# A2R-Lab/GBD-PCG

Measured on AMD Instinct MI355X. Metric: PCG iterations/sec and GB/s on block-tridiag SpMV, stateSize×knotPoints, higher is better.
Workload: dtype f32

## Files before the change

### gbd-pcg_amd/csrc/api.hip

```cpp
#include <hip/hip_runtime.h>

#include <cstdio>
#include <cstring>
#include <new>
#include <vector>

#include "../../include/gbdpcg.h"
#include "internal.hpp"

#ifndef GBDPCG_KKT_SKIP_L
#define GBDPCG_KKT_SKIP_L 1
#endif

using namespace gbdpcg;

struct gbdpcg_context {
    DeviceInfo dev;
    gbdpcg_path forced = GBDPCG_PATH_AUTO;
    int symmetric = 2;
    uint8_t *sym_flags = nullptr;
    size_t sym_cap = 0;
    hipError_t last_err = hipSuccess;
    uint32_t *d_iters = nullptr;
    uint8_t *d_exit = nullptr;
    uint32_t *h_iters = nullptr;
    uint8_t *h_exit = nullptr;
    uint32_t *h_done = nullptr;
    uint32_t *h_done_dev = nullptr;
    uint32_t *h_iters_dev = nullptr;
    uint8_t *h_exit_dev = nullptr;
    void *ws = nullptr;
    size_t ws_bytes = 0;
    struct PersistWs {
        uint64_t key;
        void *buf;
    };
    std::vector<PersistWs> pws;
    void *cluster_ws = nullptr;
    void *cluster_rescue = nullptr;
    void *pws_last = nullptr;
    std::vector<void *> retired;
};

struct gbdpcg_graph {
    gbdpcg_handle_t h = nullptr;
    hipGraph_t graph = nullptr;
    hipGraphExec_t exec = nullptr;
};

namespace gbdpcg {

template <typename T> int choose_vec(uint32_t n, const void *const *ptrs, int nptrs)
{
    const int cand[3] = {4, 2, 1};
// ... 174 lines not shown
    return grow_buffer(h, reinterpret_cast<void **>(&h->sym_flags), &h->sym_cap, batch);
}

template <typename T>
gbdpcg_status solve_impl(gbdpcg_handle_t h, uint32_t n, uint32_t N, uint32_t batch, const T *d_S, const T *d_Pinv,
                         const T *d_gamma, T *d_lambda, T *d_r, T *d_p, T tol, uint32_t max_iter,
                         uint32_t *d_iters, uint8_t *d_exit, hipStream_t stream, bool blocking = false,
                         uint32_t given_verdict_stride = 0, bool known_symmetric = false)
{
    if (!h || !d_S || !d_gamma || !d_lambda || !d_iters || !shape_ok(n, N, batch)) return GBDPCG_ERR_INVALID;
    if (!mappable<T>(n)) return GBDPCG_ERR_UNSUPPORTED;
    PcgArgs<T> a{d_S, d_Pinv, d_gamma, d_lambda, d_r, d_p, tol, max_iter, n, N, batch, d_iters, d_exit};
    a.cluster_ws = h->cluster_ws;
    a.rescue_vec = h->cluster_rescue;
    DEVICE_SCOPE(h);
    if (const uint32_t per = persist_slices<T>(h, n, N, batch, max_iter)) {
        const size_t ms = (size_t)3 * n * n * N, vs = (size_t)n * N;
        for (uint32_t b0 = 0; b0 < batch; b0 += per) {
            const uint32_t nb = batch - b0 < per ? batch - b0 : per;
            const gbdpcg_status st = solve_impl<T>(h, n, N, nb, d_S + b0 * ms, d_Pinv ? d_Pinv + b0 * ms : nullptr, d_gamma + b0 * vs,
                                                   d_lambda + b0 * vs, d_r ? d_r + b0 * vs : nullptr, d_p ? d_p + b0 * vs : nullptr, tol,
                                                   max_iter, d_iters + b0, d_exit ? d_exit + b0 : nullptr, stream);
            if (st != GBDPCG_OK) return st;
        }
        return GBDPCG_OK;
    }
    const gbdpcg_path path = pick_path<T>(h, n, N, batch);
    if (path == GBDPCG_PATH_PERSISTENT || path == GBDPCG_PATH_PERSISTENT_1R) {
        hipStreamCaptureStatus cs = hipStreamCaptureStatusNone;
        const bool capturing = hipStreamIsCapturing(stream, &cs) == hipSuccess && cs != hipStreamCaptureStatusNone;
        void *pws = nullptr;
        gbdpcg_status st = get_pws(h, sizeof(T), n, N, batch, persist_total_bytes<T>(h, n, N, batch), !capturing, &pws);
        if (st != GBDPCG_OK) return st;
        a.rescue_vec = static_cast<unsigned char *>(pws) + persist_rescue_offset<T>(n, N, batch);
        HIP_TRY(h, launch_pcg_persist<T>(h->dev, a, pws, stream, path == GBDPCG_PATH_PERSISTENT_1R));
    } else if (path == GBDPCG_PATH_FUSED) {
        const bool cluster_only = cluster_members<T>(n, N) != 0 && !resident_sym_shape<T>(n, N);
        bool has_sym = h->symmetric != 0 && d_Pinv != nullptr && !cluster_only && fused_has_symmetric<T>(h->dev, n, N, batch);
        const uint32_t members = cluster_members<T>(n, N);
        const bool one_cluster_round = members != 0 && (uint64_t)batch * members <= (uint64_t)h->dev.num_cus &&
                                       max_iter < (1u << 18) &&
                                       !(reinterpret_cast<uintptr_t>(d_S) % 8) && !(d_Pinv && reinterpret_cast<uintptr_t>(d_Pinv) % 8);
        if (h->symmetric == 2 && one_cluster_round) has_sym = false;
        if (has_sym && h->symmetric == 2 && known_symmetric) {
            a.symmetric = true;
            HIP_TRY(h, launch_pcg_fused<T>(h->dev, a, stream));
        } else if (has_sym && h->symmetric == 2 && given_verdict_stride) {
            a.sel_stride = given_verdict_stride;
            a.sel = h->sym_flags;
            a.symmetric = true;
            a.want = 1;
            HIP_TRY(h, launch_pcg_fused<T>(h->dev, a, stream));
            a.symmetric = false;
            a.want = 0;
            HIP_TRY(h, launch_pcg_fused<T>(h->dev, a, stream));
        } else if (has_sym && h->symmetric == 2) {
            const uint32_t vpp = check_pair_chunks<T>(n, N);
            const bool aligned16 = !((reinterpret_cast<uintptr_t>(d_S) | reinterpret_cast<uintptr_t>(d_Pinv)) % 16);
            const size_t need_flags = (size_t)batch * (vpp && aligned16 ? vpp : 1);
            if (need_flags > h->sym_cap) {
                hipStreamCaptureStatus cs = hipStreamCaptureStatusNone;
                if (hipStreamIsCapturing(stream, &cs) == hipSuccess && cs != hipStreamCaptureStatusNone)
                    return GBDPCG_ERR_ALLOC;
                gbdpcg_status st = ensure_sym_flags(h, need_flags);
                if (st != GBDPCG_OK) return st;
            }
            hipError_t cerr = hipSuccess;
            uint32_t stride = 1;
            if (vpp && launch_check_symmetric_pair<T>(n, N, batch, d_S, d_Pinv, h->sym_flags, stream, &cerr, &stride)) {
                HIP_TRY(h, cerr);
            } else {
                stride = 1;
                HIP_TRY(h, launch_check_symmetric<T>(h->dev, n, N, batch, d_S, h->sym_flags, false, stream));
                HIP_TRY(h, launch_check_symmetric<T>(h->dev, n, N, batch, d_Pinv, h->sym_flags, true, stream));
            }
            a.sel_stride = stride;
            a.sel = h->sym_flags;
            a.symmetric = true;
            a.want = 1;
            HIP_TRY(h, launch_pcg_fused<T>(h->dev, a, stream));
            a.symmetric = false;
            a.want = 0;
            HIP_TRY(h, launch_pcg_fused<T>(h->dev, a, stream));
        } else {
            a.symmetric = has_sym && h->symmetric == 1;
            HIP_TRY(h, launch_pcg_fused<T>(h->dev, a, stream));
        }
    } else {
        const size_t need = split_workspace_bytes<T>(n, N, batch);
        if (need > h->ws_bytes) {
            hipStreamCaptureStatus cs = hipStreamCaptureStatusNone;
            if (hipStreamIsCapturing(stream, &cs) == hipSuccess && cs != hipStreamCaptureStatusNone)
                return GBDPCG_ERR_ALLOC;
            gbdpcg_status st = ensure_ws(h, need);
            if (st != GBDPCG_OK) return st;
        }
        const volatile uint32_t *poll = nullptr;
        if (blocking && h->h_done_dev) {
            h->h_done[0] = 0;
            h->h_done[1] = 0;
            a.host_done = h->h_done_dev;
            poll = h->h_done;
        }
        HIP_TRY(h, launch_pcg_split<T>(h->dev, a, h->ws, stream, poll));
    }
    return GBDPCG_OK;
}

template <typename T>
gbdpcg_status spmv_impl(gbdpcg_handle_t h, uint32_t n, uint32_t N, uint32_t batch, const T *d_M, const T *d_x,
                        T *d_y, hipStream_t stream)
{
    if (!h || !d_M || !d_x || !d_y || !shape_ok(n, N, batch)) return GBDPCG_ERR_INVALID;
    if (!mappable<T>(n)) return GBDPCG_ERR_UNSUPPORTED;
    DEVICE_SCOPE(h);
    SpmvArgs<T> a{d_M, d_x, d_y, n, N, batch};
    a.symmetric = h->symmetric == 1;
    HIP_TRY(h, launch_spmv<T>(h->dev, a, stream));
    return GBDPCG_OK;
}

template <typename T> size_t verdict_bytes(uint32_t n, uint32_t N, uint32_t batch)
{
    const uint32_t a = check_pair_chunks<T>(n, N), b = pinv_verdict_chunks<T>(n, N, GBDPCG_PINV_STAIR);
    const uint32_t m = a > b ? a : b;
    return (size_t)batch * (m ? m : 1);
}

template <typename T>
gbdpcg_status form_pinv_solve_impl(gbdpcg_handle_t h, uint32_t n, uint32_t N, uint32_t batch, const T *d_S, T *d_Pinv,
                                   gbdpcg_pinv_kind kind, const T *d_gamma, T *d_lambda, T *d_r, T *d_p, T tol,
                                   uint32_t max_iter, uint32_t *d_iters, uint8_t *d_exit, hipStream_t stream)
{
    if (!h || !d_S || !d_Pinv || !d_gamma || !d_lambda || !d_iters || !shape_ok(n, N, batch) || (int)kind < 0 ||
        (int)kind > 2)
        return GBDPCG_ERR_INVALID;
    if (!mappable<T>(n)) return GBDPCG_ERR_UNSUPPORTED;
    DEVICE_SCOPE(h);
    uint32_t stride = 0;
    if (h->symmetric == 2 && pick_path<T>(h, n, N, batch) == GBDPCG_PATH_FUSED &&
        fused_has_symmetric<T>(h->dev, n, N, batch))
        stride = pinv_verdict_chunks<T>(n, N, (int)kind);
    if (stride) {
        const size_t need = verdict_bytes<T>(n, N, batch);
        if (need > h->sym_cap) {
            hipStreamCaptureStatus cs = hipStreamCaptureStatusNone;
            if (hipStreamIsCapturing(stream, &cs) == hipSuccess && cs != hipStreamCaptureStatusNone) return GBDPCG_ERR_ALLOC;
            gbdpcg_status st = ensure_sym_flags(h, need);
            if (st != GBDPCG_OK) return st;
        }
    }
    HIP_TRY(h, launch_form_pinv<T>(h->dev, n, N, batch, d_S, d_Pinv, (int)kind, stream, stride ? h->sym_flags : nullptr));
    return solve_impl<T>(h, n, N, batch, d_S, d_Pinv, d_gamma, d_lambda, d_r, d_p, tol, max_iter, d_iters, d_exit, stream,
                         false, stride);
}

template <typename T>
gbdpcg_status solve_blocking_impl(gbdpcg_handle_t h, uint32_t n, uint32_t N, const T *d_S, const T *d_Pinv,
                                  const T *d_gamma, T *d_lambda, T *d_r, T *d_p, T tol, uint32_t max_iter,
                                  uint32_t *h_iters, uint8_t *h_exit)
{
    if (!h) return GBDPCG_ERR_INVALID;
    hipStream_t s = nullptr;
    const bool direct = h->h_iters_dev != nullptr;
    gbdpcg_status st = solve_impl<T>(h, n, N, 1, d_S, d_Pinv, d_gamma, d_lambda, d_r, d_p, tol, max_iter,
                                     direct ? h->h_iters_dev : h->d_iters, direct ? h->h_exit_dev : h->d_exit, s, true);
    if (st != GBDPCG_OK) return st;
    if (!direct) {
        HIP_TRY(h, hipMemcpyAsync(h->h_iters, h->d_iters, sizeof(uint32_t), hipMemcpyDeviceToHost, s));
        HIP_TRY(h, hipMemcpyAsync(h->h_exit, h->d_exit, sizeof(uint8_t), hipMemcpyDeviceToHost, s));
    }
    HIP_TRY(h, hipStreamSynchronize(s));
    if (h_iters) *h_iters = *h->h_iters;
    if (h_exit) *h_exit = *h->h_exit;
    return GBDPCG_OK;
}

template <typename T>
gbdpcg_status solve_host_impl(gbdpcg_handle_t h, uint32_t n, uint32_t N, const T *h_S, const T *h_Pinv,
// ... 612 lines not shown
```

### gbd-pcg_amd/csrc/internal.hpp

```cpp
#pragma once

#include <hip/hip_runtime.h>
#include <stdint.h>
#include <stddef.h>

namespace gbdpcg {

struct DeviceInfo {
    int device = 0;
    int num_cus = 256;
    size_t lds_per_cu = 160 * 1024;
    size_t lds_per_wg_max = 160 * 1024;
};

constexpr uint32_t kItersGaveUp = 0xffffffffu;

template <typename A> __device__ __forceinline__ bool pcg_takes(const A &a, uint32_t prob)
{
    if (!a.sel) return true;
    bool sym = true;
    for (uint32_t c = 0; c < a.sel_stride; ++c) sym &= a.sel[(size_t)prob * a.sel_stride + c] == 1;
    return sym == (a.want == 1);
}

template <typename A>
__device__ __forceinline__ unsigned long long pcg_takes_mask(const A &a, uint32_t first, uint32_t step, uint32_t count, uint32_t lane)
{
    if (!a.sel) return count >= 64 ? ~0ull : ((1ull << count) - 1ull);
    bool mine = false;
    if (lane < count) {
        const size_t prob = (size_t)first + (size_t)lane * step;
        bool sym = true;
        for (uint32_t c = 0; c < a.sel_stride; ++c) sym &= a.sel[prob * a.sel_stride + c] == 1;
        mine = sym == (a.want == 1);
    }
    return __ballot(mine);
}

template <typename T> struct SpmvArgs {
    const T *M;
    const T *x;
    T *y;
    uint32_t n, N, batch;
    bool symmetric = false;
};

template <typename T> struct PcgArgs {
    const T *S;
    const T *Pinv;
    const T *gamma;
    T *lambda;
    T *r;
    T *p;
    T tol;
    uint32_t max_iter;
    uint32_t n, N, batch;
    uint32_t *iters;
    uint8_t *max_iter_exit;
    bool symmetric = false;
    const uint8_t *sel = nullptr;
    uint8_t want = 0;
    uint32_t sel_stride = 1;
    uint32_t *host_done = nullptr;
    void *cluster_ws = nullptr;
    void *rescue_vec = nullptr;
    bool rescue_off = false;
};

template <typename T> int choose_vec(uint32_t n, const void *const *ptrs, int nptrs);

#define GBDPCG_SPECIALIZED_N(X) X(2) X(4) X(6) X(8) X(10) X(12) X(13) X(14) X(16) X(18) X(20) X(24) X(36)

template <typename T, int NCT> constexpr int best_v()
{
    for (int V : {4, 2, 1})
        if ((size_t)V * sizeof(T) <= 16 && NCT % V == 0 && NCT / V <= 64) return V;
    return 1;
}

template <typename T> hipError_t launch_spmv(const DeviceInfo &dev, const SpmvArgs<T> &a, hipStream_t s);

template <typename T> size_t fused_lds_bytes(uint32_t n, uint32_t N, uint32_t waves);
template <typename T> bool fused_fits(const DeviceInfo &dev, uint32_t n, uint32_t N);
template <typename T> hipError_t launch_pcg_fused(const DeviceInfo &dev, const PcgArgs<T> &a, hipStream_t s);

template <typename T> bool resident_shape(uint32_t n, uint32_t N);
template <typename T> void resident_prepare(uint32_t n, uint32_t N);
template <typename T>
bool launch_pcg_resident(const DeviceInfo &dev, const PcgArgs<T> &a, hipStream_t s, hipError_t *err);
template <typename T> bool resident_sym_shape(uint32_t n, uint32_t N);
template <typename T>
bool launch_pcg_resident_sym(const DeviceInfo &dev, const PcgArgs<T> &a, hipStream_t s, hipError_t *err);

template <typename T> uint32_t cluster_members(uint32_t n, uint32_t N);
size_t cluster_workspace_bytes(const DeviceInfo &dev);
size_t cluster_rescue_bytes(const DeviceInfo &dev);
template <typename T>
bool launch_pcg_cluster(const DeviceInfo &dev, const PcgArgs<T> &a, hipStream_t s, hipError_t *err);

template <typename T> size_t split_workspace_bytes(uint32_t n, uint32_t N, uint32_t batch);
template <typename T>
hipError_t launch_pcg_split(const DeviceInfo &dev, const PcgArgs<T> &a, void *workspace, hipStream_t s,
                            const volatile uint32_t *host_done_poll = nullptr);

template <typename T>
uint32_t persist_knots_per_wg(const DeviceInfo &dev, uint32_t n, uint32_t N, uint32_t batch, bool one_reduction = false);
template <typename T> size_t persist_workspace_bytes(uint32_t n, uint32_t N, uint32_t batch);
template <typename T> size_t persist_rescue_bytes(uint32_t n, uint32_t N, uint32_t batch);
template <typename T>
hipError_t launch_pcg_persist(const DeviceInfo &dev, const PcgArgs<T> &a, void *workspace, hipStream_t s,
                              bool one_reduction = false);
template <typename T>
hipError_t launch_pcg_persist_b(const PcgArgs<T> &a, void *workspace, hipStream_t s, bool one_reduction, uint32_t K);
template <typename T>
hipError_t launch_pcg_persist_c(const PcgArgs<T> &a, void *workspace, hipStream_t s, bool one_reduction, uint32_t K);

template <typename T>
hipError_t launch_check_symmetric(const DeviceInfo &dev, uint32_t n, uint32_t N, uint32_t batch, const T *M,
                                  uint8_t *flags, bool and_into, hipStream_t s);
hipError_t launch_fill_bytes(uint8_t *p, uint8_t v, size_t count, hipStream_t s);
hipError_t launch_fill_words(uint32_t *p, uint32_t v, size_t count, hipStream_t s);
template <typename T>
bool launch_check_symmetric_pair(uint32_t n, uint32_t N, uint32_t batch, const T *A, const T *B, uint8_t *flags,
                                 hipStream_t s, hipError_t *err, uint32_t *verdicts_per_problem = nullptr);
template <typename T> uint32_t check_pair_chunks(uint32_t n, uint32_t N);
template <typename T> bool fused_has_symmetric(const DeviceInfo &dev, uint32_t n, uint32_t N, uint32_t batch);

template <typename T>
hipError_t launch_form_pinv(const DeviceInfo &dev, uint32_t n, uint32_t N, uint32_t batch, const T *S,
                            T *Pinv, int kind, hipStream_t s, uint8_t *verdicts = nullptr, bool s_symmetric = false);
template <typename T> uint32_t pinv_verdict_chunks(uint32_t n, uint32_t N, int kind);

template <typename T>
hipError_t launch_form_schur(const DeviceInfo &dev, uint32_t nx, uint32_t nu, uint32_t N, uint32_t batch, const T *G, const T *C,
                             const T *g, const T *c, T *S, T *gamma, T *Ginv, hipStream_t s);
template <typename T>
hipError_t launch_recover_primal(const DeviceInfo &dev, uint32_t nx, uint32_t nu, uint32_t N, uint32_t batch, const T *Ginv,
                                 const T *C, const T *g, const T *lambda, T *z, hipStream_t s);
template <typename T> bool schur_shape_ok(const DeviceInfo &dev, uint32_t nx, uint32_t nu);

}
```

### gbd-pcg_amd/csrc/pcg_resident_sym.hip

```cpp
#include <cstdlib>

#include "bt_device.hpp"
#include "bt_sym.hpp"
#include "internal.hpp"

#ifndef GBDPCG_RS_TILE_NT
#define GBDPCG_RS_TILE_NT 1
#endif
#ifndef GBDPCG_RS_PREFETCH
#define GBDPCG_RS_PREFETCH 1
#endif
#ifndef GBDPCG_RS_LINEAR_PAIRS
#define GBDPCG_RS_LINEAR_PAIRS 0
#endif

namespace gbdpcg {

template <int NCT> struct SymResGeom {
    static constexpr uint32_t N_ = NCT;
    static constexpr uint32_t QUADS = N_;
    static constexpr uint32_t WAVES = 8, GROUPS = 8, SLOTS = 2;
    static constexpr uint32_t THREADS = WAVES * 64;
    static constexpr uint32_t MAX_KNOTS = WAVES * GROUPS * SLOTS;
    static constexpr uint32_t P0_LDS_QUADS = 2;
// ... 165 lines not shown
            a10 = __builtin_elementwise_fma(v2f{v.x, v.y}, xr, a10);
            a11 = __builtin_elementwise_fma(v2f{v.z, v.w}, xr, a11);
            const v2f tp = __builtin_elementwise_fma(v2f{v.z, v.w}, v2f{o1.y, o1.y}, v2f{v.x, v.y} * v2f{o1.x, o1.x});
            tt1[2 * j] = tp.x;
            tt1[2 * j + 1] = tp.y;
        }
        asm volatile("" : "+v"(a00), "+v"(a01), "+v"(a10), "+v"(a11) : : "memory");
        __builtin_amdgcn_sched_barrier(0);
    }
    y0[0] = a00.x + a00.y; y0[1] = a01.x + a01.y;
    y1[0] = a10.x + a10.y; y1[1] = a11.x + a11.y;
}

__device__ __forceinline__ void symres_reduce_scatter14(float (&t)[14], uint32_t lane, float (&out)[2])
{
    float u0, u1, u2, u3, u4, u5, u6 = 0.f, u7 = 0.f;
#define LO(u, a) "v_add_f32_dpp %" #u ", %" #a ", %" #a " row_half_mirror row_mask:0xf bank_mask:0x5\n"
#define HI(u, a) "v_add_f32_dpp %" #u ", %" #a ", %" #a " row_half_mirror row_mask:0xf bank_mask:0xa\n"
    asm volatile("s_nop 1\n" LO(0, 8) HI(0, 16) LO(1, 9) HI(1, 17) LO(2, 10) HI(2, 18) LO(3, 11) HI(3, 19) LO(4, 12) HI(4, 20)
                 LO(5, 13) HI(5, 21) LO(6, 14) LO(7, 15)
                 : "=&v"(u0), "=&v"(u1), "=&v"(u2), "=&v"(u3), "=&v"(u4), "=&v"(u5), "+v"(u6), "+v"(u7)
                 : "v"(t[0]), "v"(t[1]), "v"(t[2]), "v"(t[3]), "v"(t[4]), "v"(t[5]), "v"(t[6]), "v"(t[7]), "v"(t[8]),
                   "v"(t[9]), "v"(t[10]), "v"(t[11]), "v"(t[12]), "v"(t[13]));
#undef LO
#undef HI
#define D(i) "v_add_f32_dpp %" #i ", %" #i ", %" #i " quad_perm:[2,3,0,1] row_mask:0xf bank_mask:0xf\n"
    asm volatile("s_nop 1\n" D(0) D(1) D(2) D(3) D(4) D(5) D(6) D(7)
                 : "+v"(u0), "+v"(u1), "+v"(u2), "+v"(u3), "+v"(u4), "+v"(u5), "+v"(u6), "+v"(u7));
#undef D
    const bool b1 = (lane & 2u) != 0;
    float w0 = b1 ? u4 : u0, w1 = b1 ? u5 : u1, w2 = b1 ? u6 : u2, w3 = b1 ? u7 : u3;
#define D(i) "v_add_f32_dpp %" #i ", %" #i ", %" #i " quad_perm:[1,0,3,2] row_mask:0xf bank_mask:0xf\n"
    asm volatile("s_nop 1\n" D(0) D(1) D(2) D(3) : "+v"(w0), "+v"(w1), "+v"(w2), "+v"(w3));
#undef D
    const bool b0 = (lane & 1u) != 0;
    out[0] = b0 ? w2 : w0;
    out[1] = b0 ? w3 : w1;
}

template <int NCT>
__device__ __forceinline__ void symres_touch(const float *M, uint32_t N, uint32_t slot, uint32_t lds_dump)
{
    constexpr uint32_t row_bytes = 2 * NCT * NCT * 4, steps = (row_bytes + 63) / 64 + 1;
    const uint32_t k = slot / steps, j = slot - k * steps;
    const uint32_t kk = k < N ? k : 0u;
    uint32_t off = j * 64;
    if (off > row_bytes - 4) off = row_bytes - 4;
    const uintptr_t addr = reinterpret_cast<uintptr_t>(M) + ((size_t)kk * 3 * NCT * NCT + NCT * NCT) * 4 + off;
    unsigned keep;
    asm volatile("s_mov_b32 %0, m0\n\ts_mov_b32 m0, %2\n\ts_nop 0\n\tglobal_load_lds_dword %1, off\n\ts_mov_b32 m0, %0"
                 : "=&s"(keep) : "v"(addr), "s"(lds_dump) : "memory");
}

__device__ __forceinline__ void symres_dma_dword(const float *base, uint32_t off, uint32_t lds_addr)
{
    unsigned keep;
    asm volatile("s_mov_b32 %0, m0\n\ts_mov_b32 m0, %3\n\ts_nop 0\n\tglobal_load_lds_dword %2, %1\n\ts_mov_b32 m0, %0"
                 : "=&s"(keep) : "s"(base), "v"(off), "s"(lds_addr) : "memory");
}

#ifdef GBDPCG_RS_STAMPS
#define GBDPCG_RS_STAMP(IDX)                                                                                             \
    if (tid == 0 && a.cluster_ws && rs_round < 8)                                                                        \
        (reinterpret_cast<unsigned long long *>(a.cluster_ws) + 1024)[(blockIdx.x * 8 + rs_round) * 8 + (IDX)] = __builtin_amdgcn_s_memrealtime();
#else
#define GBDPCG_RS_STAMP(IDX)
#endif

template <int NCT, bool STAGED>
__global__ __launch_bounds__(512) void pcg_resident_sym_kernel(PcgArgs<float> a)
{
    using G = SymResGeom<NCT>;
    static_assert(G::THREADS == 512, "launch bounds above assume 8 waves");
    static_assert(NCT == 14, "the reduce-scatter is written for 7 live lanes x 2 rows");
    constexpr uint32_t n = NCT, WAVES = G::WAVES;
    extern __shared__ __attribute__((aligned(16))) unsigned char smem_raw[];
    float *smem = reinterpret_cast<float *>(smem_raw);

    const uint32_t N = a.N, len = n * N;
    const uint32_t tid = threadIdx.x, lane = tid & 63u;
    const uint32_t wave = __builtin_amdgcn_readfirstlane(tid >> 6);
    const uint32_t padded = align16<float>((N + 3) * n);
    float *region = smem + (wave * G::GROUPS + (lane >> 3)) * G::REGION;
    float4 *lt0 = reinterpret_cast<float4 *>(smem + G::REGIONS_FLOATS) + tid;
    float *xa = smem + G::TILE_LDS_FLOATS, *xb = xa + padded;
    float *zs = xb + padded;
    float *red0 = zs + padded, *red1 = red0 + WAVES;
    float *ls = red1 + WAVES;
    const uint32_t dump = (uint32_t)(uintptr_t)(ls + align16<float>(len));

    const size_t mstride = (size_t)3 * n * n * N;

    for (uint32_t i = tid; i < padded; i += G::THREADS) zs[i] = 0.f;
    __syncthreads();

    unsigned long long takes = 0;
    uint32_t takes_from = 0;
#ifdef GBDPCG_RS_STAMPS
    uint32_t rs_round = 0xffffffffu;
#endif
    for (uint32_t prob = blockIdx.x, pi = 0; prob < a.batch; prob += gridDim.x, ++pi) {
#ifdef GBDPCG_RS_STAMPS
        ++rs_round;
#endif
        GBDPCG_RS_STAMP(0)
        if (pi == 0 || pi - takes_from >= 64) {
            const uint32_t left = (a.batch - prob + gridDim.x - 1) / gridDim.x;
            takes = pcg_takes_mask(a, prob, gridDim.x, left < 64 ? left : 64u, lane);
            takes_from = pi;
        }
        if (!((takes >> (pi - takes_from)) & 1ull)) continue;
        uint32_t lane_o = tid & 63u;
        asm volatile("" : "+v"(lane_o));
        const uint32_t rp = lane_o & 7u;
        const uint32_t grp = lane_o >> 3;
    #if GBDPCG_RS_LINEAR_PAIRS
        const uint32_t k0 = 2 * (wave * G::GROUPS + grp), k1 = k0 + 1;
    #else
        const uint32_t k0 = 2 * (16 * (wave >> 1) + 4 * (grp & 3u) + 2 * (wave & 1u) + (grp >> 2)), k1 = k0 + 1;
    #endif
        const bool live0 = rp < n / 2 && k0 < N, live1 = rp < n / 2 && k1 < N;
        const uint32_t row0 = (live0 ? k0 * n + rp * 2 : 0u), row1 = (live1 ? k1 * n + rp * 2 : 0u);
        const uint32_t xo0 = n + (live0 ? k0 : 0u) * n;
        float4_alias *ltw = reinterpret_cast<float4_alias *>(smem + wave * G::GROUPS * G::REGION) + lane_o;
        const uint32_t zo1 = n + (live1 ? k1 + 1 : 0u) * n + rp * 2;
        const uint32_t zo0 = n + (live0 ? k0 : 0u) * n + rp * 2;
        const uint32_t own0 = live0 ? n + row0 : 0u, own1 = live1 ? n + row1 : 0u;
        const float *S = a.S + prob * mstride;
        const float *P = a.Pinv + prob * mstride;
        const size_t voff = (size_t)prob * len;
        for (uint32_t q = wave; q * 64 < len; q += WAVES) {
            const uint32_t e = q * 64 + lane_o;
            if (e < len) {
                symres_dma_dword(a.lambda + voff, e * 4, (uint32_t)(uintptr_t)(ls + q * 64));
                symres_dma_dword(a.lambda + voff, e * 4, (uint32_t)(uintptr_t)(xa + n + q * 64));
                symres_dma_dword(a.gamma + voff, e * 4, (uint32_t)(uintptr_t)(xb + n + q * 64));
            }
        }

        SymResTile<NCT> s0, s1, p0;
        if constexpr (STAGED) {
            const uint32_t l8 = rp;
            const bool g0 = k0 < N, g1 = k1 < N;
            SymResStage<NCT> sa, sb, sc, sd;
            symres_stage_issue<NCT>(S, k0, g0, l8, sa);
            symres_stage_issue<NCT>(S, k1, g1, l8, sb);
            symres_stage_issue<NCT>(P, k0, g0, l8, sc);
            symres_stage_issue<NCT>(P, k1, g1, l8, sd);
            __builtin_amdgcn_sched_barrier(0);
            GBDPCG_RS_STAMP(1)
            symres_stage_park<NCT>(sa, region, l8, g0, g0 && k0 != N - 1);
            symres_stage_pick<NCT>(region, rp, live0, s0);
            __builtin_amdgcn_sched_barrier(0);
            symres_stage_park<NCT>(sb, region, l8, g1, g1 && k1 != N - 1);
            symres_stage_pick<NCT>(region, rp, live1, s1);
            __builtin_amdgcn_sched_barrier(0);
            symres_stage_park<NCT>(sc, region, l8, g0, g0 && k0 != N - 1);
            symres_stage_pick<NCT>(region, rp, live0, p0);
            __builtin_amdgcn_sched_barrier(0);
            symres_stage_park<NCT>(sd, region, l8, g1, g1 && k1 != N - 1);
            {
                SymResTile<NCT> p1;
                symres_stage_pick<NCT>(region, rp, live1, p1);
                asm volatile("" ::: "memory");
// ... 95 lines not shown
        __syncthreads();

        const uint32_t nprob = prob + gridDim.x;
        constexpr uint32_t pf_steps = (2 * n * n * 4 + 63) / 64 + 1;
        const uint32_t pf_per_matrix = GBDPCG_RS_PREFETCH && nprob < a.batch ? (N * pf_steps + G::THREADS - 1) / G::THREADS : 0u;
        uint32_t pf = 0;
#define GBDPCG_SYMRES_PREFETCH()                                                                              \
        if (pf < pf_per_matrix) {                                                                             \
            symres_touch<NCT>(a.S + nprob * mstride, N, pf * G::THREADS + tid, dump);                         \
            symres_touch<NCT>(a.Pinv + nprob * mstride, N, pf * G::THREADS + tid, dump);                      \
            ++pf;                                                                                             \
        }

        uint32_t iter = 0;
        bool max_iter_exit = true;
        GBDPCG_RS_STAMP(4)
        for (; iter < a.max_iter; ++iter) {
            GBDPCG_SYMRES_PREFETCH()
            GBDPCG_SYMRES_PRODUCT(s0, 0, s1, false, xa, part)
            const float2 pa0 = *xa0, pa1 = *xa1, la0 = *ls0, la1 = *ls1, ra0 = *xb0, ra1 = *xb1;
            float den;
            GBDPCG_SYMRES_SUM(red0, den)
            const float alpha = eta / den;
            if (live0) {
                *ls0 = make_float2(fma_t(alpha, pa0.x, la0.x), fma_t(alpha, pa0.y, la0.y));
                *xb0 = make_float2(fma_t(-alpha, y[0][0], ra0.x), fma_t(-alpha, y[0][1], ra0.y));
            }
            if (live1) {
                *ls1 = make_float2(fma_t(alpha, pa1.x, la1.x), fma_t(alpha, pa1.y, la1.y));
                *xb1 = make_float2(fma_t(-alpha, y[1][0], ra1.x), fma_t(-alpha, y[1][1], ra1.y));
            }
            __syncthreads();
            GBDPCG_SYMRES_PRODUCT(p0, G::P0_LDS_QUADS, p0, true, xb, part)
            const float2 pb0 = *xa0, pb1 = *xa1;
            float eta_new;
            GBDPCG_SYMRES_SUM(red1, eta_new)
            if (fabsf(eta_new) < a.tol) {
                ++iter;
                max_iter_exit = false;
                break;
            }
            const float beta = eta_new / eta;
            eta = eta_new;
            if (live0) *xa0 = make_float2(fma_t(beta, pb0.x, y[0][0]), fma_t(beta, pb0.y, y[0][1]));
            if (live1) *xa1 = make_float2(fma_t(beta, pb1.x, y[1][0]), fma_t(beta, pb1.y, y[1][1]));
            __syncthreads();
        }
#undef GBDPCG_SYMRES_SUM
#undef GBDPCG_SYMRES_PRODUCT
#undef GBDPCG_SYMRES_MV
#undef GBDPCG_SYMRES_FINISH_Y

        GBDPCG_RS_STAMP(5)
        while (pf < pf_per_matrix) { GBDPCG_SYMRES_PREFETCH() }
#undef GBDPCG_SYMRES_PREFETCH

        __syncthreads();
        for (uint32_t i = tid; i < len; i += G::THREADS) {
            a.lambda[voff + i] = ls[i];
            if (a.r) a.r[voff + i] = xb[n + i];
            if (a.p) a.p[voff + i] = xa[n + i];
        }
        if (tid == 0) {
            a.iters[prob] = iter;
            if (a.max_iter_exit) a.max_iter_exit[prob] = max_iter_exit ? 1 : 0;
        }
        __syncthreads();
        GBDPCG_RS_STAMP(6)
    }
    asm volatile("s_waitcnt vmcnt(0)" ::: "memory");
}

template <typename T> bool resident_sym_shape(uint32_t n, uint32_t N)
{
    static const bool off = getenv("GBDPCG_NO_RESIDENT_SYM") != nullptr;
    if (off || sizeof(T) != 4 || n != 14) return false;
    return N <= SymResGeom<14>::MAX_KNOTS;
}

static size_t resident_sym_lds(uint32_t n, uint32_t N)
{
    return ((size_t)SymResGeom<14>::TILE_LDS_FLOATS + 3 * (size_t)align16<float>((N + 3) * n) +
            2 * SymResGeom<14>::WAVES + align16<float>(N * n)) * sizeof(float) + 256;
}

template <typename T>
bool launch_pcg_resident_sym(const DeviceInfo &dev, const PcgArgs<T> &a, hipStream_t s, hipError_t *err)
{
    if constexpr (sizeof(T) == 4) {
        if (!a.symmetric || !a.Pinv || !resident_sym_shape<T>(a.n, a.N)) return false;
        if ((reinterpret_cast<uintptr_t>(a.S) % 8) || (reinterpret_cast<uintptr_t>(a.Pinv) % 8)) return false;
        const size_t lds = resident_sym_lds(a.n, a.N);
        if (lds > dev.lds_per_wg_max) return false;
        static const bool no_staging = getenv("GBDPCG_RS_DIRECT_LOADS") != nullptr;
        const bool staged = !no_staging && !((reinterpret_cast<uintptr_t>(a.S) | reinterpret_cast<uintptr_t>(a.Pinv)) % 16);
        auto kern = staged ? pcg_resident_sym_kernel<14, true> : pcg_resident_sym_kernel<14, false>;
        *err = hipFuncSetAttribute(reinterpret_cast<const void *>(kern), hipFuncAttributeMaxDynamicSharedMemorySize, (int)lds);
        if (*err != hipSuccess) return true;
        uint32_t grid = (uint32_t)dev.num_cus;
        if (grid > a.batch) grid = a.batch;
        hipLaunchKernelGGL(kern, dim3(grid), dim3(SymResGeom<14>::THREADS), lds, s, a);
        *err = hipGetLastError();
        return true;
    } else {
        return false;
    }
}

template bool resident_sym_shape<float>(uint32_t, uint32_t);
template bool resident_sym_shape<double>(uint32_t, uint32_t);
template bool launch_pcg_resident_sym<float>(const DeviceInfo &, const PcgArgs<float> &, hipStream_t, hipError_t *);
template bool launch_pcg_resident_sym<double>(const DeviceInfo &, const PcgArgs<double> &, hipStream_t, hipError_t *);

}
```

### gbd-pcg_amd/csrc/schur.hip

```cpp
#include <cstdlib>

#include "bt_device.hpp"
#include "internal.hpp"

#ifndef GBDPCG_SCHUR_SKIP
#define GBDPCG_SCHUR_SKIP 0
#endif

#ifdef GBDPCG_SCHUR_STAMPS
#define SCHUR_STAMP(i) do { if (stamp_now) { unsigned long long t_; asm volatile("s_memtime %0\n\ts_waitcnt lgkmcnt(0)" : "=s"(t_) :: "memory"); st[i] = t_; } } while (0)
#else
#define SCHUR_STAMP(i) do { } while (0)
#endif

namespace gbdpcg {

namespace {

__device__ __forceinline__ void wave_sync()
{
    __builtin_amdgcn_fence(__ATOMIC_ACQ_REL, "wavefront");
    __builtin_amdgcn_wave_barrier();
}

// ... 309 lines not shown
__device__ __forceinline__ void quad_eliminate(T (&Qc)[NX], T (&Rc)[NU], uint32_t l, F &&between)
{
    if constexpr (J < NX) {
        quad_pivot<J, NX>(Qc, l);
        if constexpr (J < NU) quad_pivot<J, NU>(Rc, l);
        between(J);
        quad_eliminate<J + 1, NX, NU>(Qc, Rc, l, between);
    }
}

template <typename T, int NX, int NU> struct QuadGeom {
    static constexpr uint32_t CP = 16;
    static constexpr uint32_t SG = NX * NX + NU * NU, SC = NX * NX + NX * NU, SV = NX + NU;
    static constexpr uint32_t DW = sizeof(T) / 4;
    static constexpr uint32_t pad(uint32_t elems) { return (elems * DW + 63) / 64 * 64 / DW; }
    static constexpr uint32_t RG = 0, RC = RG + pad(4 * SG), Rg = RC + pad(4 * SC), Rc = Rg + pad(4 * SV), RAW_P = Rc + pad(4 * NX);
    static constexpr bool SINGLE = GBDPCG_SCHUR_SINGLE != 0;
    static constexpr uint32_t WSL = (SINGLE ? 1 : 2) * RAW_P;
    static constexpr uint32_t TSL = WSL + 5 * (NX + 1) * CP;
    static constexpr uint32_t VSL = TSL + 5 * NX * CP;
    static constexpr uint32_t DSL = SINGLE ? RC : VSL + 5 * CP;
    static constexpr uint32_t GAM = SINGLE ? VSL + 5 * CP : DSL + 4 * NX * NX;
    static constexpr uint32_t ZER = (GAM + 4 * NX + 3) & ~3u;
    static constexpr uint32_t TOTAL = ZER + CP;
    static constexpr uint32_t SROW = 3 * NX * NX;
};

}

template <typename T, int NX, int NU>
__device__ __forceinline__ void schur_form_quad_body(uint32_t N, uint32_t run, uint32_t waves, const T *__restrict__ G,
                                                     const T *__restrict__ C, const T *__restrict__ g, const T *__restrict__ c,
                                                     T *__restrict__ S, T *__restrict__ gamma, T *__restrict__ Ginv)
{
    using Q = QuadGeom<T, NX, NU>;
    static_assert(NX <= 15 && NU <= 15 && NU <= NX, "one knot per 16-lane quarter, one spare lane for the vector");
    constexpr uint32_t CP = Q::CP, DW = sizeof(T) / 4;
    extern __shared__ __attribute__((aligned(16))) unsigned char smem_raw[];
    T *lds = reinterpret_cast<T *>(smem_raw);
    uint32_t lane = threadIdx.x;
    asm volatile("" : "+v"(lane));
    __builtin_assume(lane < 64);
    const uint32_t l = lane & 15u, qd = lane >> 4;
    const uint32_t w = blockIdx.x;
    if (w >= waves) return;
    const uint32_t rpp = N / run;
    const uint32_t prob = w / rpp, j_start = (w - prob * rpp) * run;
    const KktDims d(NX, NU, N);
    const T *Gp = G + (size_t)prob * d.szG, *Cp = C + (size_t)prob * d.szC, *gp = g + (size_t)prob * d.szg, *cp = c + (size_t)prob * d.szc;

    constexpr uint32_t SW = GBDPCG_SCHUR_ST4 && Q::SROW % 4 == 0 ? 4 : 1;
    constexpr uint32_t ST_I = SW * sizeof(T) > 16 ? SW * sizeof(T) / 16 : 1;
    constexpr uint32_t OUT_T = (4 * Q::SROW / SW + 63) / 64, GI_T = (4 * Q::SG / SW + 63) / 64;
    constexpr uint32_t S_STORES = OUT_T * ST_I + 1, GI_STORES = GI_T * ST_I;
    static_assert((4 * Q::SROW) % SW == 0 && Q::SROW % SW == 0 && (4 * Q::SG) % SW == 0, "whole groups");
    typedef T OutV __attribute__((ext_vector_type(SW == 4 ? 4 : 2), aligned(sizeof(T))));
    uint32_t src[OUT_T][SW];
#pragma unroll
    for (uint32_t t = 0; t < OUT_T; ++t)
#pragma unroll
        for (uint32_t u = 0; u < SW; ++u) {
            const uint32_t e0 = (t * 64 + lane) * SW + u, e = e0 < 4 * Q::SROW ? e0 : 0u;
            const uint32_t q = e / Q::SROW, i = e - q * Q::SROW, slot = i / (NX * NX), ii = i - slot * (NX * NX), cc = ii / NX, r = ii - cc * NX;
            src[t][u] = slot == 0 ? Q::WSL + q * (NX + 1) * CP + cc * CP + r
                        : slot == 1 ? Q::DSL + q * NX * NX + ii
                                    : Q::WSL + (q + 1) * (NX + 1) * CP + r * CP + cc;
        }
    auto put = [&](T *dst, const T (&v)[SW]) {
        if constexpr (SW == 1) {
            dst[0] = v[0];
        } else {
            OutV o;
#pragma unroll
            for (uint32_t u = 0; u < SW; ++u) o[u] = v[u];
#if GBDPCG_SCHUR_NT
            __builtin_nontemporal_store(o, reinterpret_cast<OutV *>(dst));
#else
            *reinterpret_cast<OutV *>(dst) = o;
#endif
        }
    };
    for (uint32_t i = lane; i < (NX + 1) * CP; i += 64) lds[Q::WSL + 4 * (NX + 1) * CP + i] = T(0);
    for (uint32_t i = lane; i < NX * CP; i += 64) lds[Q::TSL + 4 * NX * CP + i] = T(0);
    if (lane < CP) lds[Q::VSL + 4 * CP + lane] = T(0);
    if (lane < CP) lds[Q::ZER + lane] = T(0);

    const uint32_t batch = waves / rpp;
    auto request = [&](uint32_t jb, uint32_t b) {
        const uint32_t base = (uint32_t)(uintptr_t)(lds + b * Q::RAW_P);
        {
            const size_t eG = (size_t)prob * d.szG + (size_t)jb * Q::SG + Q::pad(4 * Q::SG), eC = (size_t)prob * d.szC + (size_t)jb * Q::SC + Q::pad(4 * Q::SC);
            const size_t eg = (size_t)prob * d.szg + (size_t)jb * Q::SV + Q::pad(4 * Q::SV), ec = (size_t)prob * d.szc + (size_t)jb * NX + Q::pad(4 * NX);
            if (eG <= (size_t)batch * d.szG && eC <= (size_t)batch * d.szC && eg <= (size_t)batch * d.szg && ec <= (size_t)batch * d.szc) {
                const uint32_t lo = lane * 4;
                dma_region<4 * Q::SG * DW>(Gp + (size_t)jb * Q::SG, lo, base + Q::RG * DW * 4);
                dma_region<4 * Q::SC * DW>(Cp + (size_t)jb * Q::SC, lo, base + Q::RC * DW * 4);
                dma_region<4 * Q::SV * DW>(gp + (size_t)jb * Q::SV, lo, base + Q::Rg * DW * 4);
                dma_region<4 * NX * DW>(cp + (size_t)jb * NX, lo, base + Q::Rc * DW * 4);
                return;
            }
        }
        const uint32_t lim_G = (uint32_t)(d.szG - (size_t)jb * Q::SG) * DW, lim_C = jb < N - 1 ? (uint32_t)(d.szC - (size_t)jb * Q::SC) * DW : 0u;
        const uint32_t lim_g = (uint32_t)(d.szg - (size_t)jb * Q::SV) * DW;
        const T *sG = Gp + (size_t)jb * Q::SG, *sC = Cp + (size_t)jb * Q::SC, *sg = gp + (size_t)jb * Q::SV, *sc = cp + (size_t)jb * NX;
#pragma unroll
        for (uint32_t o = 0; o < 4 * Q::SG * DW; o += 64)
            if (o + lane < 4 * Q::SG * DW && o + lane < lim_G) dma_dword(sG, (o + lane) * 4, base + (Q::RG * DW + o) * 4);
#pragma unroll
        for (uint32_t o = 0; o < 4 * Q::SC * DW; o += 64)
            if (o + lane < 4 * Q::SC * DW && o + lane < lim_C) dma_dword(sC, (o + lane) * 4, base + (Q::RC * DW + o) * 4);
#pragma unroll
        for (uint32_t o = 0; o < 4 * Q::SV * DW; o += 64)
            if (o + lane < 4 * Q::SV * DW && o + lane < lim_g) dma_dword(sg, (o + lane) * 4, base + (Q::Rg * DW + o) * 4);
        const uint32_t lim_c = (uint32_t)(d.szc - (size_t)jb * NX) * DW;
#pragma unroll
        for (uint32_t o = 0; o < 4 * NX * DW; o += 64)
            if (o + lane < 4 * NX * DW && o + lane < lim_c) dma_dword(sc, (o + lane) * 4, base + (Q::Rc * DW + o) * 4);
    };

    const bool pre = j_start != 0;
    const uint32_t j_first = pre ? j_start - 4 : j_start, j_end = j_start + run;
    request(j_first, 0);
    uint32_t b = 0, stores_since_request = 0;
    bool pending = false;
    T *So_prev = S, *gam_prev = gamma;
#ifdef GBDPCG_SCHUR_STAMPS
    unsigned long long st[12] = {};
#endif
    constexpr bool SINGLE = Q::SINGLE;
    T outv[OUT_T][SW], outg = T(0);
#pragma unroll
    for (uint32_t t = 0; t < OUT_T; ++t)
#pragma unroll
        for (uint32_t u = 0; u < SW; ++u) outv[t][u] = T(0);
    for (uint32_t jb = j_first; jb < j_end; jb += 4, b ^= (SINGLE ? 0u : 1u)) {
        const bool emit = jb >= j_start;
#ifdef GBDPCG_SCHUR_STAMPS
        const bool stamp_now = blockIdx.x == 0 && jb == 20;
#endif
        SCHUR_STAMP(0);
        static_assert(S_STORES + GI_STORES <= 63, "vmcnt is a 6-bit counter");
        switch ((GBDPCG_SCHUR_SKIP & 4) || SINGLE ? 0u : stores_since_request) {
        case S_STORES + GI_STORES: asm volatile("s_waitcnt vmcnt(%0) lgkmcnt(0)" ::"n"(S_STORES + GI_STORES) : "memory"); break;
        case S_STORES: asm volatile("s_waitcnt vmcnt(%0) lgkmcnt(0)" ::"n"(S_STORES) : "memory"); break;
        case GI_STORES: asm volatile("s_waitcnt vmcnt(%0) lgkmcnt(0)" ::"n"(GI_STORES) : "memory"); break;
        default: asm volatile("s_waitcnt vmcnt(0) lgkmcnt(0)" ::: "memory"); break;
        }
        stores_since_request = 0;
        SCHUR_STAMP(1);
        if (!SINGLE && jb + 4 < j_end && !(GBDPCG_SCHUR_SKIP & 8)) request(jb + 4, b ^ 1u);
        SCHUR_STAMP(2);
        T *raw = lds + b * Q::RAW_P;
        T *rQ = raw + Q::RG + qd * Q::SG, *rR = rQ + NX * NX, *rA = raw + Q::RC + qd * Q::SC, *rB = rA + NX * NX;
        if (jb + 4 >= N) {
            const uint32_t ql = N - 1 - jb;
            T *lR = raw + Q::RG + ql * Q::SG + NX * NX, *lA = raw + Q::RC + ql * Q::SC, *lr = raw + Q::Rg + ql * Q::SV + NX;
            for (uint32_t i = lane; i < NU * NU; i += 64) lR[i] = (i / NU == i % NU) ? T(1) : T(0);
            for (uint32_t i = lane; i < Q::SC; i += 64) lA[i] = T(0);
            if (lane < NU) lr[lane] = T(0);
            for (uint32_t q = ql + 1; q < 4; ++q) {
                T *dQ = raw + Q::RG + q * Q::SG, *dR = dQ + NX * NX, *dA = raw + Q::RC + q * Q::SC;
                for (uint32_t i = lane; i < NX * NX; i += 64) dQ[i] = (i / NX == i % NX) ? T(1) : T(0);
                for (uint32_t i = lane; i < NU * NU; i += 64) dR[i] = (i / NU == i % NU) ? T(1) : T(0);
                for (uint32_t i = lane; i < Q::SC; i += 64) dA[i] = T(0);
            }
        }
        wave_sync();
        T Qc[NX], Rc[NU];
        {
            const T *zero = lds + Q::ZER;
            const T *pq = l < NX ? rQ + l * NX : (l == NX ? raw + Q::Rg + qd * Q::SV : zero);
            const T *pr = l < NU ? rR + l * NU : (l == NU ? raw + Q::Rg + qd * Q::SV + NX : zero);
#pragma unroll
            for (uint32_t r = 0; r < NX; ++r) Qc[r] = pq[r];
#pragma unroll
            for (uint32_t r = 0; r < NU; ++r) Rc[r] = pr[r];
        }
        SCHUR_STAMP(3);
        constexpr uint32_t PER = (OUT_T + NX - 2) / (NX - 1);
        static_assert(PER * (NX - 1) >= OUT_T, "the last pivot's slot is gamma's");
        if (pending) stores_since_request += S_STORES;
        auto drain = [&](uint32_t J) {
#pragma unroll
            for (uint32_t t = J * PER; t < (J + 1) * PER && t < OUT_T; ++t)
                if (J + 1 < NX && (t * 64 + lane) * SW < 4 * Q::SROW) put(So_prev + (t * 64 + lane) * SW, outv[t]);
            if (J + 1 == NX && lane < 4 * NX) gam_prev[lane] = outg;
        };
        if (!(GBDPCG_SCHUR_SKIP & 1)) {
            if (pending && !SINGLE) quad_eliminate<0, NX, NU>(Qc, Rc, l, drain);
            else quad_eliminate<0, NX, NU>(Qc, Rc, l, [](uint32_t) {});
        } else if (pending && !SINGLE) {
#pragma unroll
            for (uint32_t J = 0; J < NX; ++J) drain(J);
        }
        SCHUR_STAMP(4);
        {
            constexpr uint32_t WT = ((NX + 1) * CP + 63) / 64, TT = (NX * CP + 63) / 64;
            T cw[WT], ct[TT];
#pragma unroll
            for (uint32_t t = 0; t < WT; ++t) cw[t] = lds[Q::WSL + 4 * (NX + 1) * CP + (t * 64 + lane < (NX + 1) * CP ? t * 64 + lane : 0u)];
#pragma unroll
            for (uint32_t t = 0; t < TT; ++t) ct[t] = lds[Q::TSL + 4 * NX * CP + (t * 64 + lane < NX * CP ? t * 64 + lane : 0u)];
            const T cv = lds[Q::VSL + 4 * CP + (lane & (CP - 1))];
#pragma unroll
            for (uint32_t t = 0; t < WT; ++t)
                if (t * 64 + lane < (NX + 1) * CP) lds[Q::WSL + t * 64 + lane] = cw[t];
#pragma unroll
            for (uint32_t t = 0; t < TT; ++t)
                if (t * 64 + lane < NX * CP) lds[Q::TSL + t * 64 + lane] = ct[t];
            if (lane < CP) lds[Q::VSL + lane] = cv;
        }
        wave_sync();
        SCHUR_STAMP(5);
        if (Ginv) {
            if (l < NX) {
#pragma unroll
                for (uint32_t r = 0; r < NX; ++r) rQ[l * NX + r] = Qc[r];
            }
            if (l < NU) {
#pragma unroll
                for (uint32_t r = 0; r < NU; ++r) rR[l * NU + r] = Rc[r];
            }
        }
        T Ac[NX], Bc[NX], ar[NX], brow[NU];
        {
            const uint32_t lc = l < NX ? l : 0u, lb = l < NU ? l : 0u;
#pragma unroll
            for (uint32_t r = 0; r < NX; ++r) {
                Ac[r] = rA[lc * NX + r];
                Bc[r] = rB[lb * NX + r];
                ar[r] = rA[r * NX + lc];
            }
#pragma unroll
            for (uint32_t q = 0; q < NU; ++q) brow[q] = rB[q * NX + lc];
// ... 355 lines not shown
```

Before: 62.14 million.

## Fuse symmetry verification into resident symmetric PCG kernel, fall back per problem

Adds a VERIFY variant of the resident symmetric PCG kernel that solves each problem on the symmetric path while also checking that the stored off-diagonal blocks of S and Pinv are mirror images of each other. Problems that pass keep their results; failures are flagged in a verdict array and re-solved by the general fused kernel through the selection mask. This replaces the separate symmetry check pass plus the two-launch split with a speculative solve, at the price of extra comparison loads per block and wasted work on nonsymmetric inputs. The schur.hip change is only a rename of a constant.

New measurement: 67.96 million, median of 6. +9.4%, better.

```diff
diff --git a/gbd-pcg_amd/csrc/api.hip b/gbd-pcg_amd/csrc/api.hip
--- a/gbd-pcg_amd/csrc/api.hip
+++ b/gbd-pcg_amd/csrc/api.hip
@@ -1,5 +1,6 @@
 #include <hip/hip_runtime.h>
 
+#include <cassert>
 #include <cstdio>
 #include <cstring>
 #include <new>
@@ -280,6 +281,25 @@
             a.want = 1;
             HIP_TRY(h, launch_pcg_fused<T>(h->dev, a, stream));
             a.symmetric = false;
+            a.want = 0;
+            HIP_TRY(h, launch_pcg_fused<T>(h->dev, a, stream));
+        } else if (has_sym && h->symmetric == 2 && resident_sym_verifies<T>(h->dev, n, N, d_S, d_Pinv)) {
+            if (batch > h->sym_cap) {
+                hipStreamCaptureStatus cs = hipStreamCaptureStatusNone;
+                if (hipStreamIsCapturing(stream, &cs) == hipSuccess && cs != hipStreamCaptureStatusNone)
+                    return GBDPCG_ERR_ALLOC;
+                gbdpcg_status st = ensure_sym_flags(h, batch);
+                if (st != GBDPCG_OK) return st;
+            }
+            a.symmetric = true;
+            a.verdict_out = h->sym_flags;
+            hipError_t rerr = hipSuccess;
+            if (!launch_pcg_resident_sym_verify<T>(h->dev, a, stream, &rerr)) return GBDPCG_ERR_UNSUPPORTED;
+            HIP_TRY(h, rerr);
+            a.verdict_out = nullptr;
+            a.symmetric = false;
+            a.sel_stride = 1;
+            a.sel = h->sym_flags;
             a.want = 0;
             HIP_TRY(h, launch_pcg_fused<T>(h->dev, a, stream));
         } else if (has_sym && h->symmetric == 2) {
@@ -352,7 +372,9 @@
 {
     const uint32_t a = check_pair_chunks<T>(n, N), b = pinv_verdict_chunks<T>(n, N, GBDPCG_PINV_STAIR);
     const uint32_t m = a > b ? a : b;
-    return (size_t)batch * (m ? m : 1);
+    const size_t bytes = (size_t)batch * (m ? m : 1);
+    assert(bytes >= batch);
+    return bytes;
 }
 
 template <typename T>
diff --git a/gbd-pcg_amd/csrc/internal.hpp b/gbd-pcg_amd/csrc/internal.hpp
--- a/gbd-pcg_amd/csrc/internal.hpp
+++ b/gbd-pcg_amd/csrc/internal.hpp
@@ -61,6 +61,7 @@
     const uint8_t *sel = nullptr;
     uint8_t want = 0;
     uint32_t sel_stride = 1;
+    uint8_t *verdict_out = nullptr;
     uint32_t *host_done = nullptr;
     void *cluster_ws = nullptr;
     void *rescue_vec = nullptr;
@@ -91,6 +92,9 @@
 template <typename T> bool resident_sym_shape(uint32_t n, uint32_t N);
 template <typename T>
 bool launch_pcg_resident_sym(const DeviceInfo &dev, const PcgArgs<T> &a, hipStream_t s, hipError_t *err);
+template <typename T> bool resident_sym_verifies(const DeviceInfo &dev, uint32_t n, uint32_t N, const T *S, const T *Pinv);
+template <typename T>
+bool launch_pcg_resident_sym_verify(const DeviceInfo &dev, const PcgArgs<T> &a, hipStream_t s, hipError_t *err);
 
 template <typename T> uint32_t cluster_members(uint32_t n, uint32_t N);
 size_t cluster_workspace_bytes(const DeviceInfo &dev);
diff --git a/gbd-pcg_amd/csrc/pcg_resident_sym.hip b/gbd-pcg_amd/csrc/pcg_resident_sym.hip
--- a/gbd-pcg_amd/csrc/pcg_resident_sym.hip
+++ b/gbd-pcg_amd/csrc/pcg_resident_sym.hip
@@ -241,6 +241,29 @@
                  : "=&s"(keep) : "v"(addr), "s"(lds_dump) : "memory");
 }
 
+template <int NCT>
+__device__ __forceinline__ void symres_lcols_issue(const float *__restrict__ M, uint32_t k, uint32_t rp, bool cmp,
+                                                   float4 (&l)[NCT / 2])
+{
+    constexpr uint32_t n = NCT;
+    const float4 *src = reinterpret_cast<const float4 *>(M + (cmp ? (size_t)(k + 1) * 3 * n * n + 2 * rp * n : (size_t)0));
+#pragma unroll
+    for (uint32_t m = 0; m < n / 2; ++m) l[m] = src[m];
+}
+template <int NCT>
+__device__ __forceinline__ bool symres_r_differs(const float4 (&r)[NCT / 2], const float4 (&l)[NCT / 2], bool cmp)
+{
+    constexpr uint32_t n = NCT;
+    auto comp = [](const float4 &v, uint32_t i) { return i == 0 ? v.x : i == 1 ? v.y : i == 2 ? v.z : v.w; };
+    uint32_t diff = 0;
+#pragma unroll
+    for (uint32_t e = 0; e < 2 * n; ++e) {
+        const uint32_t hi = e / n, c = e % n;
+        diff |= __builtin_bit_cast(uint32_t, comp(l[e / 4], e % 4)) ^ __builtin_bit_cast(uint32_t, comp(r[c / 2], 2 * hi + (c & 1)));
+    }
+    return cmp && diff != 0;
+}
+
 __device__ __forceinline__ void symres_dma_dword(const float *base, uint32_t off, uint32_t lds_addr)
 {
     unsigned keep;
@@ -256,7 +279,7 @@
 #define GBDPCG_RS_STAMP(IDX)
 #endif
 
-template <int NCT, bool STAGED>
+template <int NCT, bool STAGED, bool VERIFY = false>
 __global__ __launch_bounds__(512) void pcg_resident_sym_kernel(PcgArgs<float> a)
 {
     using G = SymResGeom<NCT>;
@@ -277,6 +300,7 @@
     float *red0 = zs + padded, *red1 = red0 + WAVES;
     float *ls = red1 + WAVES;
     const uint32_t dump = (uint32_t)(uintptr_t)(ls + align16<float>(len));
+    uint32_t *vword = reinterpret_cast<uint32_t *>(ls + align16<float>(len)) + 64;
 
     const size_t mstride = (size_t)3 * n * n * N;
 
@@ -293,12 +317,18 @@
         ++rs_round;
 #endif
         GBDPCG_RS_STAMP(0)
-        if (pi == 0 || pi - takes_from >= 64) {
-            const uint32_t left = (a.batch - prob + gridDim.x - 1) / gridDim.x;
-            takes = pcg_takes_mask(a, prob, gridDim.x, left < 64 ? left : 64u, lane);
-            takes_from = pi;
-        }
-        if (!((takes >> (pi - takes_from)) & 1ull)) continue;
+        if constexpr (!VERIFY) {
+            if (pi == 0 || pi - takes_from >= 64) {
+                const uint32_t left = (a.batch - prob + gridDim.x - 1) / gridDim.x;
+                takes = pcg_takes_mask(a, prob, gridDim.x, left < 64 ? left : 64u, lane);
+                takes_from = pi;
+            }
+            if (!((takes >> (pi - takes_from)) & 1ull)) continue;
+        } else {
+            (void)takes;
+            (void)takes_from;
+            if (tid == 0) *vword = 1u;
+        }
         uint32_t lane_o = tid & 63u;
         asm volatile("" : "+v"(lane_o));
         const uint32_t rp = lane_o & 7u;
@@ -500,19 +530,53 @@
 #undef GBDPCG_SYMRES_FINISH_Y
 
         GBDPCG_RS_STAMP(5)
+        if constexpr (VERIFY) {
+            const bool cmp0 = live0 && k0 + 1 < N, cmp1 = live1 && k1 + 1 < N;
+            bool bad;
+            {
+                float4 l0[n / 2], l1[n / 2], r0[n / 2], r1[n / 2];
+                symres_lcols_issue<NCT>(S, k0, rp, cmp0, l0);
+                symres_lcols_issue<NCT>(S, k1, rp, cmp1, l1);
+#pragma unroll
+                for (uint32_t j = 0; j < n / 2; ++j) {
+                    r0[j] = s0.q[n / 2 + j];
+                    r1[j] = s1.q[n / 2 + j];
+                }
+                bad = symres_r_differs<NCT>(r0, l0, cmp0);
+                bad |= symres_r_differs<NCT>(r1, l1, cmp1);
+            }
+            __builtin_amdgcn_sched_barrier(0);
+            {
+                float4 l0[n / 2], l1[n / 2], r0[n / 2], r1[n / 2];
+                symres_lcols_issue<NCT>(P, k0, rp, cmp0, l0);
+                symres_lcols_issue<NCT>(P, k1, rp, cmp1, l1);
+#pragma unroll
+                for (uint32_t j = 0; j < n / 2; ++j) {
+                    r0[j] = p0.q[n / 2 + j];
+                    r1[j] = ltw[(n / 2 + j) * 64];
+                }
+                bad |= symres_r_differs<NCT>(r0, l0, cmp0);
+                bad |= symres_r_differs<NCT>(r1, l1, cmp1);
+            }
+            if (bad) *vword = 0u;
+        }
         while (pf < pf_per_matrix) { GBDPCG_SYMRES_PREFETCH() }
 #undef GBDPCG_SYMRES_PREFETCH
 
         __syncthreads();
-        for (uint32_t i = tid; i < len; i += G::THREADS) {
-            a.lambda[voff + i] = ls[i];
-            if (a.r) a.r[voff + i] = xb[n + i];
-            if (a.p) a.p[voff + i] = xa[n + i];
-        }
-        if (tid == 0) {
-            a.iters[prob] = iter;
-            if (a.max_iter_exit) a.max_iter_exit[prob] = max_iter_exit ? 1 : 0;
-        }
+        const bool keep = VERIFY ? __builtin_amdgcn_readfirstlane(*reinterpret_cast<volatile uint32_t *>(vword)) != 0u : true;
+        if (keep) {
+            for (uint32_t i = tid; i < len; i += G::THREADS) {
+                a.lambda[voff + i] = ls[i];
+                if (a.r) a.r[voff + i] = xb[n + i];
+                if (a.p) a.p[voff + i] = xa[n + i];
+            }
+            if (tid == 0) {
+                a.iters[prob] = iter;
+                if (a.max_iter_exit) a.max_iter_exit[prob] = max_iter_exit ? 1 : 0;
+            }
+        }
+        if (VERIFY && tid == 0) a.verdict_out[prob] = keep ? 1 : 0;
         __syncthreads();
         GBDPCG_RS_STAMP(6)
     }
@@ -526,23 +590,37 @@
     return N <= SymResGeom<14>::MAX_KNOTS;
 }
 
-static size_t resident_sym_lds(uint32_t n, uint32_t N)
+static size_t resident_sym_lds(uint32_t n, uint32_t N, bool verify = false)
 {
     return ((size_t)SymResGeom<14>::TILE_LDS_FLOATS + 3 * (size_t)align16<float>((N + 3) * n) +
-            2 * SymResGeom<14>::WAVES + align16<float>(N * n)) * sizeof(float) + 256;
+            2 * SymResGeom<14>::WAVES + align16<float>(N * n)) * sizeof(float) + 256 + (verify ? 16 : 0);
+}
+
+static bool resident_sym_staged(const void *S, const void *Pinv)
+{
+    static const bool no_staging = getenv("GBDPCG_RS_DIRECT_LOADS") != nullptr;
+    return !no_staging && !((reinterpret_cast<uintptr_t>(S) | reinterpret_cast<uintptr_t>(Pinv)) % 16);
 }
 
 template <typename T>
-bool launch_pcg_resident_sym(const DeviceInfo &dev, const PcgArgs<T> &a, hipStream_t s, hipError_t *err)
+bool resident_sym_verifies(const DeviceInfo &dev, uint32_t n, uint32_t N, const T *S, const T *Pinv)
+{
+    return sizeof(T) == 4 && S && Pinv && resident_sym_shape<T>(n, N) && resident_sym_staged(S, Pinv) &&
+           resident_sym_lds(n, N, true) <= dev.lds_per_wg_max;
+}
+
+template <typename T>
+static bool launch_pcg_resident_sym_impl(const DeviceInfo &dev, const PcgArgs<T> &a, hipStream_t s, hipError_t *err, bool verify)
 {
     if constexpr (sizeof(T) == 4) {
         if (!a.symmetric || !a.Pinv || !resident_sym_shape<T>(a.n, a.N)) return false;
         if ((reinterpret_cast<uintptr_t>(a.S) % 8) || (reinterpret_cast<uintptr_t>(a.Pinv) % 8)) return false;
-        const size_t lds = resident_sym_lds(a.n, a.N);
+        const size_t lds = resident_sym_lds(a.n, a.N, verify);
         if (lds > dev.lds_per_wg_max) return false;
-        static const bool no_staging = getenv("GBDPCG_RS_DIRECT_LOADS") != nullptr;
-        const bool staged = !no_staging && !((reinterpret_cast<uintptr_t>(a.S) | reinterpret_cast<uintptr_t>(a.Pinv)) % 16);
-        auto kern = staged ? pcg_resident_sym_kernel<14, true> : pcg_resident_sym_kernel<14, false>;
+        const bool staged = resident_sym_staged(a.S, a.Pinv);
+        if (verify && (!staged || !a.verdict_out)) return false;
+        auto kern = verify ? pcg_resident_sym_kernel<14, true, true>
+                           : staged ? pcg_resident_sym_kernel<14, true, false> : pcg_resident_sym_kernel<14, false, false>;
         *err = hipFuncSetAttribute(reinterpret_cast<const void *>(kern), hipFuncAttributeMaxDynamicSharedMemorySize, (int)lds);
         if (*err != hipSuccess) return true;
         uint32_t grid = (uint32_t)dev.num_cus;
@@ -555,9 +633,25 @@
     }
 }
 
+template <typename T>
+bool launch_pcg_resident_sym(const DeviceInfo &dev, const PcgArgs<T> &a, hipStream_t s, hipError_t *err)
+{
+    return launch_pcg_resident_sym_impl<T>(dev, a, s, err, false);
+}
+
+template <typename T>
+bool launch_pcg_resident_sym_verify(const DeviceInfo &dev, const PcgArgs<T> &a, hipStream_t s, hipError_t *err)
+{
+    return launch_pcg_resident_sym_impl<T>(dev, a, s, err, true);
+}
+
 template bool resident_sym_shape<float>(uint32_t, uint32_t);
 template bool resident_sym_shape<double>(uint32_t, uint32_t);
 template bool launch_pcg_resident_sym<float>(const DeviceInfo &, const PcgArgs<float> &, hipStream_t, hipError_t *);
 template bool launch_pcg_resident_sym<double>(const DeviceInfo &, const PcgArgs<double> &, hipStream_t, hipError_t *);
-
-}
+template bool resident_sym_verifies<float>(const DeviceInfo &, uint32_t, uint32_t, const float *, const float *);
+template bool resident_sym_verifies<double>(const DeviceInfo &, uint32_t, uint32_t, const double *, const double *);
+template bool launch_pcg_resident_sym_verify<float>(const DeviceInfo &, const PcgArgs<float> &, hipStream_t, hipError_t *);
+template bool launch_pcg_resident_sym_verify<double>(const DeviceInfo &, const PcgArgs<double> &, hipStream_t, hipError_t *);
+
+}
diff --git a/gbd-pcg_amd/csrc/schur.hip b/gbd-pcg_amd/csrc/schur.hip
--- a/gbd-pcg_amd/csrc/schur.hip
+++ b/gbd-pcg_amd/csrc/schur.hip
@@ -385,7 +385,7 @@
     constexpr uint32_t SW = GBDPCG_SCHUR_ST4 && Q::SROW % 4 == 0 ? 4 : 1;
     constexpr uint32_t ST_I = SW * sizeof(T) > 16 ? SW * sizeof(T) / 16 : 1;
     constexpr uint32_t OUT_T = (4 * Q::SROW / SW + 63) / 64, GI_T = (4 * Q::SG / SW + 63) / 64;
-    constexpr uint32_t S_STORES = OUT_T * ST_I + 1, GI_STORES = GI_T * ST_I;
+    constexpr uint32_t SG_STORES = OUT_T * ST_I + 1, GI_STORES = GI_T * ST_I;
     static_assert((4 * Q::SROW) % SW == 0 && Q::SROW % SW == 0 && (4 * Q::SG) % SW == 0, "whole groups");
     typedef T OutV __attribute__((ext_vector_type(SW == 4 ? 4 : 2), aligned(sizeof(T))));
     uint32_t src[OUT_T][SW];
@@ -472,10 +472,10 @@
         const bool stamp_now = blockIdx.x == 0 && jb == 20;
 #endif
         SCHUR_STAMP(0);
-        static_assert(S_STORES + GI_STORES <= 63, "vmcnt is a 6-bit counter");
+        static_assert(SG_STORES + GI_STORES <= 63, "vmcnt is a 6-bit counter");
         switch ((GBDPCG_SCHUR_SKIP & 4) || SINGLE ? 0u : stores_since_request) {
-        case S_STORES + GI_STORES: asm volatile("s_waitcnt vmcnt(%0) lgkmcnt(0)" ::"n"(S_STORES + GI_STORES) : "memory"); break;
-        case S_STORES: asm volatile("s_waitcnt vmcnt(%0) lgkmcnt(0)" ::"n"(S_STORES) : "memory"); break;
+        case SG_STORES + GI_STORES: asm volatile("s_waitcnt vmcnt(%0) lgkmcnt(0)" ::"n"(SG_STORES + GI_STORES) : "memory"); break;
+        case SG_STORES: asm volatile("s_waitcnt vmcnt(%0) lgkmcnt(0)" ::"n"(SG_STORES) : "memory"); break;
         case GI_STORES: asm volatile("s_waitcnt vmcnt(%0) lgkmcnt(0)" ::"n"(GI_STORES) : "memory"); break;
         default: asm volatile("s_waitcnt vmcnt(0) lgkmcnt(0)" ::: "memory"); break;
         }
@@ -512,7 +512,7 @@
         SCHUR_STAMP(3);
         constexpr uint32_t PER = (OUT_T + NX - 2) / (NX - 1);
         static_assert(PER * (NX - 1) >= OUT_T, "the last pivot's slot is gamma's");
-        if (pending) stores_since_request += S_STORES;
+        if (pending) stores_since_request += SG_STORES;
         auto drain = [&](uint32_t J) {
 #pragma unroll
             for (uint32_t t = J * PER; t < (J + 1) * PER && t < OUT_T; ++t)
```
